# soedinglab/plass

Hardware: AMD Instinct MI355X
Metric: read-overlaps/s per assembly iteration (higher is better)
Workload: dtype u8/u64 (integer hash, byte compare; f32 ratios)

## Files before the change

### plass_amd/csrc/kmermatch.hip

```cpp
#include "common.hpp"
#include "device_utils.hpp"
#include "host_util.hpp"
#include "linepart.hpp"
#include "ref_rules.hpp"
#include "xxh64_u64.hpp"
#include <algorithm>
#include <memory>
#include <type_traits>
#include <cstdlib>
#include <climits>
#include <cstring>

namespace plasship {

#include "kmermatch_extract.hpp"
#include "kmermatch_group.hpp"
#include "kmermatch_repsort.hpp"
}
using namespace plasship;

namespace {

struct Timer {
    plasship_ctx *ctx; int slot;
    void start(int s) { slot = s; (void) hipEventRecord(ctx->ev[s], ctx->stream); }
    float stop(int s2) { (void) hipEventRecord(ctx->ev[s2], ctx->stream); (void) hipEventSynchronize(ctx->ev[s2]); float ms = 0; (void) hipEventElapsedTime(&ms, ctx->ev[slot], ctx->ev[s2]); return ms; }
};

static inline unsigned gridFor(uint64_t n, unsigned block, unsigned cap = 65535u * 8) {
    uint64_t g = (n + block - 1) / block; if (g < 1) g = 1; if (g > cap) g = cap; return (unsigned) g;
}
static int ceilLog2(uint64_t x) { int b = 0; while ((1ULL << b) < x) b++; return b; }

__global__ void lastRunInfoKernel(const unsigned long long *__restrict__ maxRT, const uint64_t *__restrict__ slotOff, const uint32_t *__restrict__ len,
                                  uint32_t n, unsigned long long *__restrict__ out) {
    const unsigned long long m = *maxRT;
    const uint32_t t = (uint32_t) (m & 0xFFFFFFFFull);
    out[0] = m;
    if (t < n) { out[1] = slotOff[t]; out[2] = slotOff[t + 1]; out[3] = len[t]; } else { out[1] = out[2] = out[3] = 0; }
}

template <bool LONG>
__global__ void countBadIdsKernel(const void *recs, uint64_t n, uint32_t nSeq, unsigned long long *out) {
    const Rec<LONG> *g = reinterpret_cast<const Rec<LONG> *>(recs);
    unsigned long long bad = 0, sen = 0;
    for (uint64_t i = (uint64_t) blockIdx.x * blockDim.x + threadIdx.x; i < n; i += (uint64_t) gridDim.x * blockDim.x) {
        const Rec<LONG> r = g[i];
        if (isSentinel(r)) sen++; else if (r.id >= nSeq) bad++;
    }
    if (bad) atomicAdd(&out[0], bad);
    if (sen) atomicAdd(&out[1], sen);
}
template <bool LONG>
static void traceBadIds(plasship_ctx *ctx, const char *what, const void *recs, uint64_t n, uint32_t nSeq) {
    if (!traceOn()) return;
    DevBuf d; unsigned long long h[2] = {0, 0};
    if (d.alloc(16) != hipSuccess) return;
    (void) hipMemsetAsync(d.p, 0, 16, ctx->stream);
    hipLaunchKernelGGL((countBadIdsKernel<LONG>), dim3(1024), dim3(256), 0, ctx->stream, recs, n, nSeq, d.as<unsigned long long>());
    (void) hipMemcpyAsync(h, d.p, 16, hipMemcpyDeviceToHost, ctx->stream);
    const hipError_t e = plasship::streamSync(ctx->stream);
    fprintf(stderr, "[plasship] %s: %llu records, %llu with an id out of range, %llu sentinels (%s)\n", what, (unsigned long long) n, h[0], h[1], hipGetErrorString(e));
}

__global__ void splitIdsKernel(const uint64_t *__restrict__ slotOff, uint32_t n, int W, uint64_t *__restrict__ out) {
    const uint64_t total = slotOff[n];
    for (int r = threadIdx.x; r <= W; r += blockDim.x) {
        uint32_t lo = 0, hi = n;
        if (r == W) lo = n;
        else {
            const uint64_t want = (uint64_t) (((unsigned __int128) total * (unsigned) r) / (unsigned) W);
            while (lo < hi) { const uint32_t mid = lo + (hi - lo) / 2; if (slotOff[mid] < want) lo = mid + 1; else hi = mid; }
        }
        out[r] = lo; out[W + 1 + r] = slotOff[lo];
    }
}

struct LineGeo {
    int b1 = 0, b2 = 0; uint32_t nb1 = 1, nb2 = 0, PL1 = 1, PL2 = 0;
    uint64_t totalLines = 0, nP1 = 0, cap1 = 0, maxP2 = 0, cap2 = 0;
    uint32_t lastValid = RPL;
};
static uint32_t pieceLinesFor(uint64_t lines, uint32_t nb, int numCU, uint32_t minFactor) {
    const uint64_t want = (lines + 4ull * (uint64_t) numCU - 1) / (4ull * (uint64_t) numCU);
    return (uint32_t) std::max<uint64_t>((uint64_t) nb * minFactor, std::min<uint64_t>((uint64_t) nb * 64, std::max<uint64_t>(want, 1)));
}
static LineGeo lineGeometry(uint64_t totalSlots, bool lng, int numCU, uint64_t slotsAll = 0, int W = 1) {
    LineGeo g;
    const int maxBits = lng ? 9 : 10;
    const int lw = ceilLog2((uint64_t) std::max(W, 1));
    int totalBits = std::min(2 * maxBits, std::max(lw, std::max(0, ceilLog2(((slotsAll ? slotsAll : totalSlots) + 1535) / 1536))));
    if (const char *pb = getenv("PLASSHIP_TUNE_PART_BITS")) { if (*pb) totalBits = std::min(2 * maxBits, std::max(lw, atoi(pb))); }
    g.b1 = totalBits <= maxBits ? totalBits : std::max((totalBits + 1) / 2, lw); g.b2 = totalBits - g.b1;
    g.nb1 = 1u << g.b1; g.nb2 = g.b2 ? 1u << g.b2 : 0u;
    g.totalLines = (totalSlots + RPL - 1) / RPL;
    g.lastValid = g.totalLines ? (uint32_t) (totalSlots - (g.totalLines - 1) * RPL) : (uint32_t) RPL;
    g.PL1 = pieceLinesFor(g.totalLines, g.nb1, numCU, 8);
    g.nP1 = (g.totalLines + g.PL1 - 1) / g.PL1;
    g.cap1 = std::max<uint64_t>(g.nP1 * ((uint64_t) g.PL1 + g.nb1), 1);
    if (g.nb2) {
        g.PL2 = 0xFFFFFFFFu; g.maxP2 = g.nb1; g.cap2 = g.cap1 + (uint64_t) g.nb1 * g.nb2;
    }
    return g;
}
static uint64_t repLevel1Cap(uint64_t nRec, uint64_t nSeg, uint32_t PL, uint32_t nb) {
    const uint64_t lines = (nRec + RPL - 1) / RPL + nSeg;
    return lines + (lines / PL + nSeg + 1) * (uint64_t) nb;
}

__global__ void arenaStartKernel(const uint32_t *__restrict__ lineBeg, uint32_t bpb, uint32_t gGrid, uint32_t nBuckets, uint64_t *__restrict__ arenaStart) {
    for (uint32_t j = blockIdx.x * blockDim.x + threadIdx.x; j < gGrid; j += gridDim.x * blockDim.x)
        arenaStart[j] = (uint64_t) lineBeg[std::min(j * bpb, nBuckets - 1)] * RPL;
}
__global__ void bigNeedKernel(const uint32_t *__restrict__ lineCnt, const uint32_t *__restrict__ unique, uint32_t nBuckets, uint64_t *__restrict__ need, uint32_t wordsPerEntry) {
    for (uint32_t b = blockIdx.x * blockDim.x + threadIdx.x; b < nBuckets; b += gridDim.x * blockDim.x) {
        const uint64_t c = (uint64_t) lineCnt[b] * RPL;
        uint64_t v = 0;
        if (unique[b] == AGG_NEEDS_SCRATCH) { uint64_t P = 1; while (P < c) P <<= 1; v = wordsPerEntry * P; }
        need[b] = v;
    }
}
__global__ void sumU32Kernel(const uint32_t *__restrict__ v, uint32_t n, unsigned long long *__restrict__ out) {
    unsigned long long s = 0;
    for (uint32_t i = blockIdx.x * blockDim.x + threadIdx.x; i < n; i += gridDim.x * blockDim.x) s += v[i];
    s = waveReduceSumU64(s);
    if (laneId() == 0 && s) atomicAdd(out, s);
}

template <class K> static int setDynLds(K k, size_t bytes) {
    PH_CHECK(hipFuncSetAttribute(reinterpret_cast<const void *>(k), hipFuncAttributeMaxDynamicSharedMemorySize, (int) bytes));
    return PLASSHIP_OK;
}
template <bool NUCL, bool LONG, int MODE, bool LIST, bool EXTRAS>
static int launchLinePart(plasship_ctx *ctx, const LinePartArgs &a, uint64_t nPiecesBound) {
    const size_t lds = linePartLdsBytes(a.nb, sizeof(Rec<LONG>), EXTRAS);
    const bool big = lds > 72 * 1024;
    const unsigned grid = (unsigned) std::max<uint64_t>(1, std::min<uint64_t>(nPiecesBound, (uint64_t) ctx->numCU * (big ? 1u : 2u)));
    if (big) {
        auto k = linePartKernel<NUCL, LONG, MODE, LIST, EXTRAS, 1024, 4, true>;
        const int rc = setDynLds(k, lds); if (rc) return rc;
        hipLaunchKernelGGL(k, dim3(grid), dim3(1024), lds, ctx->stream, a);
    } else {
        auto k = linePartKernel<NUCL, LONG, MODE, LIST, EXTRAS, 512, 4, true>;
        const int rc = setDynLds(k, lds); if (rc) return rc;
        hipLaunchKernelGGL(k, dim3(grid), dim3(512), lds, ctx->stream, a);
    }
    return PLASSHIP_OK;
}

static int buildLineLists(plasship_ctx *ctx, const uint32_t *dTags, uint64_t capLines, uint32_t nb, uint32_t *dCount, uint32_t *dStart, uint32_t *dCursor, uint32_t *dList) {
    hipStream_t st = ctx->stream;
    PH_CHECK(hipMemsetAsync(dCount, 0, (size_t) nb * 4, st));
    const unsigned g = (unsigned) std::max<uint64_t>(1, std::min<uint64_t>((capLines + 4095) / 4096, (uint64_t) ctx->numCU * 8));
    const unsigned gs = (unsigned) std::max<uint64_t>(1, std::min<uint64_t>((capLines + TS_CHUNK - 1) / TS_CHUNK, (uint64_t) ctx->numCU * 2));
    hipLaunchKernelGGL(tagHistKernel, dim3(g), dim3(256), 0, st, dTags, capLines, nb, dCount);
    hipLaunchKernelGGL(tagScanKernel, dim3(1), dim3(1024), 0, st, (const uint32_t *) dCount, nb, dStart, dCursor);
    hipLaunchKernelGGL(tagScatterKernel, dim3(gs), dim3(TS_BLOCK), 0, st, dTags, capLines, nb, dCursor, dList);
    return PLASSHIP_OK;
}

static bool shardOwnerFiltered(int W) { const int m = tuneInt("SHARD_EXTRACT", 0); return m == 2 || (m != 1 && W <= 4); }

constexpr int KM_RETRY_EARLY_OVERFLOW_CHECK = -1000;
struct LinesOut { void *triples = nullptr; uint64_t nTriples = 0, Nk = 0, Nm = 0; std::vector<int64_t> stalePos; uint32_t staleT = 0; float msSort1 = 0, msGroup = 0, msSort2 = 0, msPart = 0; int nPart = 1;
                  uint64_t exchangedRecordBytes = 0, exchangedTripleBytes = 0; };

constexpr uint64_t HALO_SLACK = 1u << 16;

static bool aggHistOn() { return getenv("PLASSHIP_DEBUG_AGGHIST") != nullptr; }
static int aggHistRecord(hipStream_t st, const uint32_t *dLineCnt, const uint32_t *dUnique, uint32_t nSort) {
    static int call = 0;
    std::vector<uint32_t> lc(nSort), uq(nSort);
    PH_COPY_SYNC(st, lc.data(), dLineCnt, (size_t) nSort * 4, hipMemcpyDeviceToHost);
    PH_COPY_SYNC(st, uq.data(), dUnique, (size_t) nSort * 4, hipMemcpyDeviceToHost);
    constexpr int NB = 10;
    auto bin = [](uint64_t v) { if (!v) return 0; int k = 1; uint64_t e = 64; while (k < NB - 1 && v > e) { e <<= 1; k++; } return k; };
    uint64_t hr[NB] = {}, hd[NB] = {}, sr = 0, sd = 0, mr = 0, md = 0, big = 0;
    for (uint32_t b = 0; b < nSort; b++) {
        const uint64_t r = (uint64_t) lc[b] * RPL; hr[bin(r)]++; sr += r; mr = std::max(mr, r);
        if (uq[b] == AGG_NEEDS_SCRATCH) { big++; continue; }
        hd[bin(uq[b])]++; sd += uq[b]; md = std::max<uint64_t>(md, uq[b]);
    }
    std::string s = "aggHist call " + std::to_string(call++) + " buckets " + std::to_string(nSort) + " | bins 0,<=64,<=128,...,<=8192,>8192 | slots";
    for (int k = 0; k < NB; k++) s += " " + std::to_string(hr[k]);
    s += " (mean " + std::to_string(nSort ? sr / nSort : 0) + ", max " + std::to_string(mr) + ") | distinct";
    for (int k = 0; k < NB; k++) s += " " + std::to_string(hd[k]);
    s += " (mean " + std::to_string(nSort ? sd / nSort : 0) + ", max " + std::to_string(md) + ", scratch " + std::to_string(big) + ")";
    fprintf(stderr, "%s\n", s.c_str());
    return PLASSHIP_OK;
}

constexpr int GW_BLOCK = 512; constexpr uint32_t GW_HT = 4096;
static bool groupHistOn() { return getenv("PLASSHIP_DEBUG_GROUPHIST") != nullptr; }
template <bool NUCL, bool LONG>
static int groupHistRecord(hipStream_t st, const char *kernel, uint32_t regCap, uint32_t maxKeys, uint32_t nBuckets, uint32_t bpb, const uint32_t *dFineBeg, const uint32_t *dFineCnt,
                           const uint32_t *dList, const void *dRecs, uint64_t capLines) {
    typedef Rec<LONG> R;
    static int call = 0;
    std::vector<uint32_t> beg(nBuckets), cnt(nBuckets);
    if (nBuckets) { PH_COPY_SYNC(st, beg.data(), dFineBeg, (size_t) nBuckets * 4, hipMemcpyDeviceToHost); PH_COPY_SYNC(st, cnt.data(), dFineCnt, (size_t) nBuckets * 4, hipMemcpyDeviceToHost); }
    uint64_t listEnd = 0;
    for (uint32_t b = 0; b < nBuckets; b++) if (cnt[b]) listEnd = std::max<uint64_t>(listEnd, (uint64_t) beg[b] + cnt[b]);
    if (listEnd > capLines) { setError("kmermatch: groupHist: a bucket's line list ends behind the list"); return PLASSHIP_ERR_DEVICE; }
    std::vector<uint32_t> list(listEnd); std::vector<R> recs((size_t) capLines * RPL);
    if (listEnd) PH_COPY_SYNC(st, list.data(), dList, (size_t) listEnd * 4, hipMemcpyDeviceToHost);
    if (listEnd) PH_COPY_SYNC(st, recs.data(), dRecs, recs.size() * sizeof(R), hipMemcpyDeviceToHost);
    enum { EMPTY = 0, REGS = 1, BIG = 2 };
    static const char *const CLS[3] = {"empty", "regs", "big"};
    auto cls = [&](uint32_t b) { const uint64_t n = (uint64_t) cnt[b] * RPL; return n == 0 ? EMPTY : (regCap == 0 || n <= regCap) ? REGS : BIG; };
    uint64_t maxPos = 0, over = 0, maxDistinct = 0, maxSub = nBuckets ? 1 : 0, multiSub = 0, pairs[3][3] = {}, bigFirst = 0, bigLater = 0, records = 0;
    std::vector<unsigned long long> keys, per;
    for (uint32_t b = 0; b < nBuckets; b++) {
        const uint64_t n = (uint64_t) cnt[b] * RPL;
        maxPos = std::max(maxPos, n);
        if (cls(b) == BIG) { over++; (b % bpb == 0 ? bigFirst : bigLater)++; }
        if (b % bpb != 0) pairs[cls(b - 1)][cls(b)]++;
        keys.clear();
        for (uint32_t l = 0; l < cnt[b]; l++) {
            const uint64_t line = list[beg[b] + l];
            if (line >= capLines) { setError("kmermatch: groupHist: a line list entry is out of range"); return PLASSHIP_ERR_DEVICE; }
            for (int i = 0; i < RPL; i++) { const R &r = recs[line * RPL + i]; if (!(r.kmer == ~0ULL && r.id == 0xFFFFFFFFu)) keys.push_back(NUCL ? (r.kmer | BIT63) : r.kmer); }
        }
        records += keys.size();
        std::sort(keys.begin(), keys.end()); keys.erase(std::unique(keys.begin(), keys.end()), keys.end());
        maxDistinct = std::max<uint64_t>(maxDistinct, keys.size());
        uint32_t nSub = 1;
        for (;; nSub *= 2) {
            per.assign(nSub, 0);
            for (const unsigned long long K : keys) per[(uint32_t) (((K * 0xD6E8FEB86659FD93ULL) >> 40) % nSub)]++;
            if (*std::max_element(per.begin(), per.end()) <= maxKeys) break;
        }
        maxSub = std::max<uint64_t>(maxSub, nSub); multiSub += nSub > 1;
    }
    std::string s = "groupHist call " + std::to_string(call++) + " kernel " + kernel + " buckets " + std::to_string(nBuckets) + " bpb " + std::to_string(bpb) + " records " + std::to_string(records) +
                    " | maxPos " + std::to_string(maxPos) + " regCap " + std::to_string(regCap) + " overRegs " + std::to_string(over) + " (first " + std::to_string(bigFirst) + ", later " + std::to_string(bigLater) + ")" +
                    " | maxDistinct " + std::to_string(maxDistinct) + " maxKeys " + std::to_string(maxKeys) + " | maxSub " + std::to_string(maxSub) + " multiSub " + std::to_string(multiSub) + " | pairs";
    for (int p = 0; p < 3; p++) for (int q = 0; q < 3; q++) s += std::string(" ") + CLS[p] + ">" + CLS[q] + " " + std::to_string(pairs[p][q]);
    fprintf(stderr, "%s\n", s.c_str());
    return PLASSHIP_OK;
}

template <bool NUCL, bool LONG, bool TRIPLES, bool ORDOUT = false>
static int repSortLines(plasship_ctx *ctx, const void *in, const std::vector<std::pair<uint64_t, uint64_t>> &segs, uint64_t nIn, uint32_t nReps, uint32_t repBase, uint32_t nTargets,
                        uint64_t slackTriples, const std::function<void()> &inputConsumed, DevBuf &dOut, uint64_t &nTriples, DevBuf *dRepStartOut) {
    constexpr bool PL = TRIPLES ? NUCL : LONG;
    typedef Rec<PL> R;
    typedef typename std::conditional<ORDOUT, TripleX, Triple>::type OutT;
    hipStream_t st = ctx->stream;
    const int numCU = ctx->numCU;
    const int maxBits = PL ? 9 : 10;
    const int idBits = std::max(1, ceilLog2((uint64_t) nTargets));
    const int repBits = std::max(1, ceilLog2((uint64_t) std::max<uint32_t>(nReps, 1)));
    const int wantBits = std::min(2 * maxBits, std::max(0, ceilLog2((nIn + 511) / 512)));
    const int allowedLocal = 62 - idBits - DiagPack<LONG>::BITS;
    const int sBits = std::max(std::min(wantBits, repBits), std::max(0, repBits - allowedLocal));
    if (sBits > 2 * maxBits) { setError("kmermatch: too many sequences for the packed rep-sort key"); return PLASSHIP_ERR_UNSUPPORTED; }
    const int s1 = sBits <= maxBits ? sBits : (sBits + 1) / 2, s2 = sBits - s1;
    const uint32_t nS1 = 1u << s1, nS2 = s2 ? 1u << s2 : 0u, nSort = 1u << sBits;
    std::vector<LinePiece> hp; uint64_t outLine = 0;
    {
        uint64_t totLines = 0; for (const auto &sg : segs) totLines += (sg.second + RPL - 1) / RPL;
        const uint32_t PLr1 = pieceLinesFor(totLines, nS1, numCU, 8);
        for (const auto &sg : segs) {
            const uint64_t cnt = sg.second, lines = (cnt + RPL - 1) / RPL;
            for (uint64_t l0 = 0; l0 < lines; l0 += PLr1) {
                LinePiece pc; pc.in0 = sg.first + l0; pc.nLines = (uint32_t) std::min<uint64_t>(PLr1, lines - l0);
                pc.lastValid = (l0 + pc.nLines == lines) ? (uint32_t) (cnt - (lines - 1) * RPL) : (uint32_t) RPL;
                pc.out0 = outLine; pc.outCap = pc.nLines + nS1; pc.tagBase = 0;
                outLine += pc.outCap; hp.push_back(pc);
            }
        }
    }
    const uint32_t PLr2 = s2 ? pieceLinesFor(std::max<uint64_t>(outLine, 1), nS2, numCU, 16) : 0;
    const uint64_t maxPR2 = s2 ? std::max<uint64_t>(outLine, 1) / PLr2 + nS1 + 1 : 0;
    const uint64_t capR1 = std::max<uint64_t>(outLine, 1), capR2 = s2 ? capR1 + maxPR2 * nS2 : 0;
    const uint32_t nPR1 = (uint32_t) hp.size();
    DevBuf dR1, dRTag1, dRList1, dRPieces, dRNP, dRCnt1, dRStart1, dRCur1, dR2, dRTag2, dRList2, dRPieces2, dRNP2, dRRegBeg, dRRegEnd, dRTot2, dSortBeg, dSortCnt;
    if (dR1.alloc(capR1 * RPL * sizeof(R)) != hipSuccess || dRTag1.alloc(capR1 * 4) != hipSuccess || dRList1.alloc(capR1 * 4) != hipSuccess || dRPieces.alloc(((size_t) nPR1 + 1) * sizeof(LinePiece)) != hipSuccess ||
        dRNP.alloc(4) != hipSuccess || dRCnt1.alloc(LP_MAXB * 4) != hipSuccess || dRStart1.alloc((LP_MAXB + 1) * 4) != hipSuccess || dRCur1.alloc(LP_MAXB * 4) != hipSuccess ||
        dSortBeg.alloc((size_t) nSort * 4) != hipSuccess || dSortCnt.alloc((size_t) nSort * 4) != hipSuccess) { setError("kmermatch: out of device memory for the rep sort"); return PLASSHIP_ERR_DEVICE; }
    void *hpPinned = nPR1 ? ctxPinnedTable(ctx, (size_t) nPR1 * sizeof(LinePiece)) : nullptr;
    if (hpPinned) memcpy(hpPinned, hp.data(), (size_t) nPR1 * sizeof(LinePiece));
    if (nPR1) PH_CHECK(hipMemcpyAsync(dRPieces.p, hpPinned ? hpPinned : (const void *) hp.data(), (size_t) nPR1 * sizeof(LinePiece), hipMemcpyHostToDevice, st));
    else PH_CHECK(hipMemsetAsync(dRTag1.p, 0xFF, capR1 * 4, st));
    PH_CHECK(hipMemcpyAsync(dRNP.p, &nPR1, 4, hipMemcpyHostToDevice, st));
    LineKey rkey; rkey.rangeBits = repBits; rkey.repBase = repBase; rkey.shift = s1 ? 64 - s1 : 63; rkey.scrambleBits = repBits;
    int rc;
    {
        LinePartArgs a; memset(&a, 0, sizeof(a));
        a.in = in; a.out = dR1.p; a.tags = dRTag1.as<uint32_t>(); a.pieces = dRPieces.as<LinePiece>(); a.nPieces = dRNP.as<uint32_t>(); a.nb = nS1; a.key = rkey;
        a.direct = 1;
        rc = launchLinePart<NUCL, PL, KEY_RANGE, false, false>(ctx, a, std::max<uint32_t>(nPR1, 1)); if (rc) return rc;
// ... 796 lines not shown
```

### plass_amd/csrc/kmermatch_group.hpp

```cpp
#pragma once

constexpr int GR_BLOCK = 256;
constexpr uint32_t GR_HT = 2048;
constexpr uint32_t GR_MAXKEYS = 1536;

struct GroupArgs {
    const void *in; void *out;
    const uint64_t *bucketStart;
    const uint32_t *list, *lineBeg, *lineCnt;
    uint32_t nBuckets, bucketsPerBlock;
    uint64_t *outCount;
    int includeOnlyExtendable, covMode; float covThr;
    const unsigned long long *minKey;
    unsigned long long *maxRepTarget;
};

template <bool LONG> __device__ __forceinline__ void embedOrd(Rec<LONG> &o, uint64_t memberKmerField) {
    const uint64_t K = memberKmerField & ~BIT63;
    o.kmer |= (K & 0x7FFFFFFFull) << 32;
    o.len = (decltype(o.len)) (K >> 31);
}
template <bool LONG> __device__ __forceinline__ unsigned long long ordWordOf(const Rec<LONG> &r) {
    const uint64_t K = ((r.kmer >> 32) & 0x7FFFFFFFull) | ((uint64_t) (LONG ? (uint32_t) r.len : (uint32_t) (uint16_t) r.len) << 31);
    return (K << 1) | (r.kmer >> 63);
// ... 9 lines not shown
    __shared__ uint32_t sCursor;
    typedef Rec<LONG> R;
    const R *in = reinterpret_cast<const R *>(a.in);
    R *out = reinterpret_cast<R *>(a.out);
    const uint32_t bBegin = blockIdx.x * a.bucketsPerBlock;
    const uint32_t bEnd = min(a.nBuckets, bBegin + a.bucketsPerBlock);
    if (bBegin >= a.nBuckets) { if (threadIdx.x == 0) a.outCount[blockIdx.x] = 0; return; }
    unsigned long long written = 0;
    unsigned long long maxRT = 0;
    const uint64_t arena = LINES ? (uint64_t) a.lineBeg[bBegin] * RPL : a.bucketStart[bBegin];
    const unsigned long long firstRunKey = (NUCL && a.minKey) ? *a.minKey : 0ull;
    for (uint32_t b = bBegin; b < bEnd; b++) {
        const uint64_t s0 = LINES ? 0ull : a.bucketStart[b], s1 = LINES ? (uint64_t) a.lineCnt[b] * RPL : a.bucketStart[b + 1];
        const uint32_t lb = LINES ? a.lineBeg[b] : 0u;
        auto recAt = [&](uint64_t i) -> R { if (LINES) return in[(uint64_t) a.list[lb + (uint32_t) (i / RPL)] * RPL + (i % RPL)]; return in[i]; };
        if (s1 <= s0) continue;
        uint32_t nSub = 1;
        const unsigned long long writtenAtBucketStart = written;
        for (;;) {
            bool redo = false;
            for (uint32_t sub = 0; sub < nSub && !redo; sub++) {
                for (uint32_t i = threadIdx.x; i < GR_HT; i += GR_BLOCK) { hKey[i] = ~0ULL; hBest[i] = ~0ULL; hCnt[i] = 0; hLen[i] = 0; }
                if (threadIdx.x == 0) { sFlag[0] = 0; sFlag[1] = 0; sCursor = 0; }
                __syncthreads();
                for (uint64_t i = s0 + threadIdx.x; i < s1; i += GR_BLOCK) {
                    const R r = recAt(i);
                    if (LINES && isSentinel(r)) continue;
                    const unsigned long long K = NUCL ? (r.kmer | BIT63) : r.kmer;
                    const uint64_t hh = K * 0xD6E8FEB86659FD93ULL;
                    if (nSub > 1 && (uint32_t) ((hh >> 40) % nSub) != sub) continue;
                    uint32_t slot = (uint32_t) (hh >> 32) & (GR_HT - 1);
                    for (uint32_t probe = 0; probe < GR_HT; probe++) {
                        const unsigned long long prev = atomicCAS(&hKey[slot], ~0ULL, K);
                        if (prev == ~0ULL) { atomicAdd(&sFlag[0], 1u); }
                        if (prev == ~0ULL || prev == K) { atomicAdd(&hCnt[slot], 1u); atomicMax(&hLen[slot], (uint32_t) r.len); break; }
                        slot = (slot + 1) & (GR_HT - 1);
                        if (probe == GR_HT - 1) atomicExch(&sFlag[1], 1u);
                    }
                }
                __syncthreads();
                if (sFlag[1] || sFlag[0] > GR_MAXKEYS) { redo = true; __syncthreads(); break; }
                for (uint64_t i = s0 + threadIdx.x; i < s1; i += GR_BLOCK) {
                    const R r = recAt(i);
                    if (LINES && isSentinel(r)) continue;
                    const unsigned long long K = NUCL ? (r.kmer | BIT63) : r.kmer;
                    const uint64_t hh = K * 0xD6E8FEB86659FD93ULL;
                    if (nSub > 1 && (uint32_t) ((hh >> 40) % nSub) != sub) continue;
                    uint32_t slot = (uint32_t) (hh >> 32) & (GR_HT - 1);
                    while (hKey[slot] != K) slot = (slot + 1) & (GR_HT - 1);
                    if ((uint32_t) r.len == hLen[slot]) {
                        const unsigned long long packed = ((unsigned long long) r.id << 22) | ((unsigned long long) (uint32_t) r.pos << 1) | (NUCL ? ((r.kmer >> 63) & 1ULL) : 0ULL);
                        atomicMin(&hBest[slot], packed);
                    }
                }
                __syncthreads();
                for (uint64_t i0 = s0; i0 < s1; i0 += GR_BLOCK) {
                    const uint64_t i = i0 + threadIdx.x;
                    bool keep = false; R o; memset(&o, 0, sizeof(R));
                    if (i < s1) {
                        const R r = recAt(i);
                        const unsigned long long K = NUCL ? (r.kmer | BIT63) : r.kmer;
                        const uint64_t hh = K * 0xD6E8FEB86659FD93ULL;
                        if (!(LINES && isSentinel(r)) && !(nSub > 1 && (uint32_t) ((hh >> 40) % nSub) != sub)) {
                            uint32_t slot = (uint32_t) (hh >> 32) & (GR_HT - 1);
                            while (hKey[slot] != K) slot = (slot + 1) & (GR_HT - 1);
                            if (hCnt[slot] >= 2) {
                                const unsigned long long best = hBest[slot];
                                const uint32_t repId = (uint32_t) (best >> 22);
                                const int repPos = (int) ((best >> 1) & 0x1FFFFFu);
                                const int queryLen = (int) hLen[slot];
                                const int mLen = (int) r.len, mPos = (int) r.pos;
                                int diagonal = repPos - mPos;
                                unsigned long long rId = repId;
                                if (NUCL) {
                                    bool repIsReverse = ((best & 1ULL) == 0);
                                    if (K == firstRunKey) repIsReverse = false;
                                    const bool targetIsReverse = ((r.kmer & BIT63) == 0);
                                    int qp, tp; bool qRev;
                                    if (repIsReverse && !targetIsReverse) { qp = repPos; tp = mPos; qRev = true; }
                                    else if (repIsReverse && targetIsReverse) { qp = (queryLen - 1) - repPos; tp = (mLen - 1) - mPos; qRev = false; }
                                    else if (!repIsReverse && targetIsReverse) { qp = (queryLen - 1) - repPos; tp = (mLen - 1) - mPos; qRev = true; }
                                    else { qp = repPos; tp = mPos; qRev = false; }
                                    if (!LONG) { qp = (int) (short) qp; tp = (int) (short) tp; }
                                    diagonal = qp - tp;
                                    rId = qRev ? (rId & ~BIT63) : (rId | BIT63);
                                }
                                const bool canBeExtended = diagonal < 0 || (diagonal > (queryLen - mLen));
                                const bool cov = canBeCovered(a.covThr, a.covMode, (float) queryLen, (float) mLen);
                                keep = (!a.includeOnlyExtendable && cov) || (canBeExtended && a.includeOnlyExtendable);
                                o.kmer = rId; o.id = r.id; o.len = r.len; o.pos = (decltype(o.pos)) diagonal;
                                if (NUCL) embedOrd(o, r.kmer);
                                if (keep) maxRT = max(maxRT, (unsigned long long) (((rId & ~BIT63) << 32) | (unsigned long long) r.id));
                            }
                        }
                    }
                    const unsigned long long mk = __ballot(keep);
                    const uint32_t wr = (uint32_t) __popcll(mk & ((1ULL << laneId()) - 1ULL));
                    uint32_t wbase = 0;
                    if (mk) {
                        if (laneId() == 0) wbase = atomicAdd(&sCursor, (uint32_t) __popcll(mk));
                        wbase = __shfl(wbase, 0, 64);
                    }
                    if (keep) out[arena + written + wbase + wr] = o;
                }
                __syncthreads();
                written += sCursor;
                __syncthreads();
                if (threadIdx.x == 0) sCursor = 0;
            }
            if (!redo) break;
            nSub *= 2;
            written = writtenAtBucketStart;
            __syncthreads();
        }
    }
    if (a.maxRepTarget) {
#pragma unroll
        for (int o = 32; o > 0; o >>= 1) maxRT = max(maxRT, (unsigned long long) __shfl_xor(maxRT, o, 64));
        if (laneId() == 0 && maxRT) atomicMax(a.maxRepTarget, maxRT);
    }
    if (threadIdx.x == 0) a.outCount[blockIdx.x] = written;
}

constexpr int GL_RMAX = 8;
constexpr uint32_t glMaxKeys(uint32_t HT) { return HT / 4 * 3; }
template <bool NUCL, int BLOCK, uint32_t HT, int WPE>
__global__ __launch_bounds__(BLOCK) __attribute__((amdgpu_waves_per_eu(WPE, WPE))) void groupLinesKernel(GroupArgs a) {
    __shared__ uint32_t sList[GL_RMAX * BLOCK / RPL];
    typedef Rec<false> R;
    constexpr uint32_t MAXKEYS = glMaxKeys(HT);
    __shared__ unsigned long long hKey[HT];
    __shared__ unsigned long long hBest[HT];
    __shared__ uint32_t hMulti[HT / 32];
    __shared__ uint32_t sFlag[2];
    __shared__ uint32_t sCursor[2];
    const R *in = reinterpret_cast<const R *>(a.in);
    R *out = reinterpret_cast<R *>(a.out);
    const uint32_t bBegin = blockIdx.x * a.bucketsPerBlock;
    const uint32_t bEnd = min(a.nBuckets, bBegin + a.bucketsPerBlock);
    if (bBegin >= a.nBuckets) { if (threadIdx.x == 0) a.outCount[blockIdx.x] = 0; return; }
    unsigned long long written = 0;
    unsigned long long maxRT = 0;
    const uint64_t arena = (uint64_t) a.lineBeg[bBegin] * RPL;
    const unsigned long long firstRunKey = (NUCL && a.minKey) ? *a.minKey : 0ull;
    const R none = [] { R r; r.kmer = ~0ULL; r.id = 0xFFFFFFFFu; r.len = 0; r.pos = 0; return r; }();
    R rg[GL_RMAX];
    uint32_t nNext = 0, lbNext = 0;
    auto fetch = [&](uint32_t b, bool fromLds) {
        nNext = (b < bEnd) ? a.lineCnt[b] * RPL : 0u; lbNext = (b < bEnd) ? a.lineBeg[b] : 0u;
        if (nNext && nNext <= (uint32_t) GL_RMAX * BLOCK) {
#pragma unroll
            for (int j = 0; j < GL_RMAX; j++) {
                const uint32_t i = (uint32_t) j * BLOCK + threadIdx.x;
                const uint32_t le = fromLds ? sList[i / RPL] : a.list[lbNext + i / RPL];
                rg[j] = (i < nNext) ? in[(uint64_t) le * RPL + (i % RPL)] : none;
            }
        }
    };
    uint32_t par = 0;
    fetch(bBegin, false);
    for (uint32_t b = bBegin; b < bEnd; b++) {
        const uint32_t n = nNext;
        const uint32_t lb = lbNext;
        if (n == 0) { fetch(b + 1, false); continue; }
        uint32_t leAhead = 0; bool aheadStored = false;
        if (b + 1 < bEnd) { const uint32_t nl = a.lineCnt[b + 1]; if (threadIdx.x < nl && nl <= (uint32_t) GL_RMAX * BLOCK / RPL) leAhead = a.list[a.lineBeg[b + 1] + threadIdx.x]; }
        auto recAt = [&](uint32_t i) -> R { return in[(uint64_t) a.list[lb + i / RPL] * RPL + (i % RPL)]; };
        const bool inRegs = n <= (uint32_t) GL_RMAX * BLOCK;
        bool fetched = false;
        auto phaseA = [&](const R &r, uint32_t nSub, uint32_t sub) {
            bool claimed = false, full = false;
            const unsigned long long K = NUCL ? (r.kmer | BIT63) : r.kmer;
            const uint64_t hh = K * 0xD6E8FEB86659FD93ULL;
            if (!isSentinel(r) && !(nSub > 1 && (uint32_t) ((hh >> 40) % nSub) != sub)) {
                uint32_t slot = (uint32_t) (hh >> 32) & (HT - 1);
                full = true;
                for (uint32_t probe = 0; probe < HT; probe++) {
                    const unsigned long long prev = atomicCAS(&hKey[slot], ~0ULL, K);
                    if (prev == ~0ULL || prev == K) {
                        claimed = (prev == ~0ULL);
                        if (!claimed) atomicOr(&hMulti[slot >> 5], 1u << (slot & 31));
                        const unsigned long long packed = ((unsigned long long) (0x7FFFu - (uint32_t) r.len) << 48) | ((unsigned long long) r.id << 16) |
                                                          ((unsigned long long) ((uint32_t) r.pos & 0x7FFFu) << 1) | (NUCL ? ((r.kmer >> 63) & 1ULL) : 0ULL);
                        atomicMin(&hBest[slot], packed);
                        full = false;
                        break;
                    }
                    slot = (slot + 1) & (HT - 1);
                }
            }
            const unsigned long long cm = __ballot(claimed);
            if (cm && laneId() == 0) atomicAdd(&sFlag[0], (uint32_t) __popcll(cm));
            if (full) atomicExch(&sFlag[1], 1u);
        };
        auto phaseC = [&](const R &r, uint32_t nSub, uint32_t sub) {
            bool keep = false; R o; o.kmer = 0; o.id = 0; o.len = 0; o.pos = 0;
            if (!isSentinel(r)) {
                const unsigned long long K = NUCL ? (r.kmer | BIT63) : r.kmer;
                const uint64_t hh = K * 0xD6E8FEB86659FD93ULL;
                if (!(nSub > 1 && (uint32_t) ((hh >> 40) % nSub) != sub)) {
                    uint32_t slot = (uint32_t) (hh >> 32) & (HT - 1);
                    while (hKey[slot] != K) slot = (slot + 1) & (HT - 1);
                    if ((hMulti[slot >> 5] >> (slot & 31)) & 1u) {
                        const unsigned long long best = hBest[slot];
                        const uint32_t repId = (uint32_t) (best >> 16);
                        const int repPos = (int) ((best >> 1) & 0x7FFFu);
                        const int queryLen = (int) (0x7FFFu - (uint32_t) (best >> 48));
                        const int mLen = (int) r.len, mPos = (int) r.pos;
                        int diagonal = repPos - mPos;
                        unsigned long long rId = repId;
                        if (NUCL) {
                            bool repIsReverse = ((best & 1ULL) == 0);
                            if (K == firstRunKey) repIsReverse = false;
                            const bool targetIsReverse = ((r.kmer & BIT63) == 0);
                            int qp, tp; bool qRev;
                            if (repIsReverse && !targetIsReverse) { qp = repPos; tp = mPos; qRev = true; }
                            else if (repIsReverse && targetIsReverse) { qp = (queryLen - 1) - repPos; tp = (mLen - 1) - mPos; qRev = false; }
                            else if (!repIsReverse && targetIsReverse) { qp = (queryLen - 1) - repPos; tp = (mLen - 1) - mPos; qRev = true; }
                            else { qp = repPos; tp = mPos; qRev = false; }
                            qp = (int) (short) qp; tp = (int) (short) tp;
                            diagonal = qp - tp;
                            rId = qRev ? (rId & ~BIT63) : (rId | BIT63);
                        }
                        const bool canBeExtended = diagonal < 0 || (diagonal > (queryLen - mLen));
                        const bool cov = canBeCovered(a.covThr, a.covMode, (float) queryLen, (float) mLen);
                        keep = (!a.includeOnlyExtendable && cov) || (canBeExtended && a.includeOnlyExtendable);
                        o.kmer = rId; o.id = r.id; o.len = r.len; o.pos = (int16_t) diagonal;
                        if (NUCL) embedOrd(o, r.kmer);
                        if (keep) maxRT = max(maxRT, (unsigned long long) (((rId & ~BIT63) << 32) | (unsigned long long) r.id));
                    }
                }
            }
            const unsigned long long mk = __ballot(keep);
            const uint32_t wr = (uint32_t) __popcll(mk & ((1ULL << laneId()) - 1ULL));
            uint32_t wbase = 0;
            if (mk) {
                if (laneId() == 0) wbase = atomicAdd(&sCursor[par], (uint32_t) __popcll(mk));
                wbase = __shfl(wbase, 0, 64);
            }
            if (keep) out[arena + written + wbase + wr] = o;
        };
        uint32_t nSub = 1;
        const unsigned long long writtenAtBucketStart = written;
        for (;;) {
            bool redo = false;
            for (uint32_t sub = 0; sub < nSub && !redo; sub++) {
                for (uint32_t i = threadIdx.x; i < HT; i += BLOCK) { hKey[i] = ~0ULL; hBest[i] = ~0ULL; if (i < HT / 32) hMulti[i] = 0; }
                if (threadIdx.x == 0) { sFlag[0] = 0; sFlag[1] = 0; sCursor[par] = 0; }
                __syncthreads();
                if (inRegs) {
#pragma unroll
                    for (int j = 0; j < GL_RMAX; j++) if ((uint32_t) j * BLOCK < n) phaseA(rg[j], nSub, sub);
                } else for (uint32_t i0 = 0; i0 < n; i0 += BLOCK) { const uint32_t i = i0 + threadIdx.x; phaseA(i < n ? recAt(i) : none, nSub, sub); }
                if (!aheadStored) { if (threadIdx.x < GL_RMAX * BLOCK / RPL) sList[threadIdx.x] = leAhead; aheadStored = true; }
                __syncthreads();
                if (sFlag[1] || sFlag[0] > MAXKEYS) { redo = true; __syncthreads(); break; }
                if (inRegs && sub + 1 == nSub) {
                    const uint32_t nN = (b + 1 < bEnd) ? a.lineCnt[b + 1] * RPL : 0u, lbN = (b + 1 < bEnd) ? a.lineBeg[b + 1] : 0u;
                    const bool nextRegs = nN && nN <= (uint32_t) GL_RMAX * BLOCK;
#pragma unroll
                    for (int j = 0; j < GL_RMAX; j++) {
                        if ((uint32_t) j * BLOCK < n) phaseC(rg[j], nSub, sub);
                        if (nextRegs) { const uint32_t i = (uint32_t) j * BLOCK + threadIdx.x; rg[j] = (i < nN) ? in[(uint64_t) sList[i / RPL] * RPL + (i % RPL)] : none; }
                    }
                    nNext = nN; lbNext = lbN; fetched = true;
                } else {
                if (inRegs) {
#pragma unroll
                    for (int j = 0; j < GL_RMAX; j++) if ((uint32_t) j * BLOCK < n) phaseC(rg[j], nSub, sub);
                } else for (uint32_t i0 = 0; i0 < n; i0 += BLOCK) { const uint32_t i = i0 + threadIdx.x; phaseC(i < n ? recAt(i) : none, nSub, sub); }
                if (sub + 1 == nSub) { fetch(b + 1, true); fetched = true; }
                }
                __syncthreads();
                written += sCursor[par];
                par ^= 1u;
            }
            if (!redo) break;
            nSub *= 2;
            written = writtenAtBucketStart;
            __syncthreads();
        }
        if (!fetched) fetch(b + 1, false);
    }
    if (a.maxRepTarget) {
#pragma unroll
        for (int o = 32; o > 0; o >>= 1) maxRT = max(maxRT, (unsigned long long) __shfl_xor(maxRT, o, 64));
        if (laneId() == 0 && maxRT) atomicMax(a.maxRepTarget, maxRT);
    }
    if (threadIdx.x == 0) a.outCount[blockIdx.x] = written;
}
```

### plass_amd/csrc/linepart.hpp

```cpp
#pragma once
#include "common.hpp"
#include "device_utils.hpp"

namespace plasship {

#define BIT63 (1ULL << 63)

template <bool LONG> struct Rec;
template <> struct __attribute__((aligned(16))) Rec<false> { uint64_t kmer; uint32_t id; uint16_t len; int16_t pos; };
template <> struct __attribute__((aligned(8))) Rec<true> { uint64_t kmer; uint32_t id; int32_t len; int32_t pos; uint32_t pad; };

template <bool LONG> __device__ __forceinline__ bool isSentinel(const Rec<LONG> &r) { return r.kmer == ~0ULL && r.id == 0xFFFFFFFFu; }

enum { KEY_HASH = 0, KEY_RANGE = 1 };
template <bool NUCL> __device__ __forceinline__ uint64_t kmerMix(uint64_t kmerField) {
    const uint64_t K = NUCL ? (kmerField & ~BIT63) : kmerField;
    uint64_t x = K * 0x9E3779B97F4A7C15ULL; x ^= x >> 29; x *= 0xBF58476D1CE4E5B9ULL; x ^= x >> 32;
    return x;
}

constexpr uint32_t VH_BINS = 2048;
template <bool NUCL> __device__ __host__ __forceinline__ uint32_t valueBin(uint64_t kmerField, int shift) {
    const uint64_t v = NUCL ? (kmerField & ~BIT63) : kmerField;
    const uint64_t b = v >> shift;
    return b < VH_BINS ? (uint32_t) b : VH_BINS - 1;
}

#ifndef PLASSHIP_RPL
#define PLASSHIP_RPL 8
#endif
constexpr int RPL = PLASSHIP_RPL;
constexpr uint32_t TAG_NONE = 0xFFFFFFFFu;
constexpr uint32_t LP_MAXB = 1024;

struct LineKey {
    int shift, rangeBits;
    uint64_t repBase;
    int scrambleBits;
};
__device__ __host__ __forceinline__ uint64_t scrambleRep(uint64_t rep, int bits) {
    uint32_t x = (uint32_t) rep;
    x = ((x >> 1) & 0x55555555u) | ((x & 0x55555555u) << 1); x = ((x >> 2) & 0x33333333u) | ((x & 0x33333333u) << 2);
    x = ((x >> 4) & 0x0F0F0F0Fu) | ((x & 0x0F0F0F0Fu) << 4); x = ((x >> 8) & 0x00FF00FFu) | ((x & 0x00FF00FFu) << 8);
    x = (x >> 16) | (x << 16);
    return (uint64_t) (x >> (32 - bits));
}
template <bool NUCL, int MODE> __device__ __forceinline__ uint32_t lineBucket(const LineKey &k, uint64_t kmerField, uint32_t nb) {
    if (MODE == KEY_HASH) return (uint32_t) (kmerMix<NUCL>(kmerField) >> k.shift) & (nb - 1);
    uint64_t r = (kmerField & ~BIT63) - k.repBase;
    if (k.scrambleBits) r = scrambleRep(r, k.scrambleBits);
    return (uint32_t) ((r << (64 - k.rangeBits)) >> k.shift) & (nb - 1);
}

struct LinePiece {
    uint64_t in0;
    uint64_t out0;
    uint32_t nLines;
    uint32_t lastValid;
    uint32_t outCap;
    uint32_t tagBase;
};

struct LinePartArgs {
    const void *in; const uint32_t *list;
    void *out; uint32_t *tags;
    const LinePiece *pieces; const uint32_t *nPieces;
    uint64_t totalLines; uint32_t lastValidAll, pieceLines;
    uint32_t *pieceOut;
    LineKey key; uint32_t nb;
    int direct;
    unsigned long long *minKey;
    uint32_t *valueHist; int valueShift;
    uint32_t keepLo, keepHi;
};

static inline size_t linePartLdsBytes(uint32_t nb, size_t recBytes, bool extras) {
    return (size_t) nb * RPL * recBytes + (size_t) nb * 8 + (extras ? VH_BINS * 4 : 0) + (size_t) nb * 2 + (size_t) nb * 4 + 16;
}

template <bool NUCL, bool LONG, int MODE, bool LIST, bool EXTRAS, int LP_BLOCK, int LP_ITEMS, bool PREFETCH>
__global__ __launch_bounds__(LP_BLOCK) void linePartKernel(LinePartArgs a) {
    constexpr int LP_TILE = LP_BLOCK * LP_ITEMS;
    typedef Rec<LONG> R;
    extern __shared__ __attribute__((aligned(16))) unsigned char lpDyn[];
    const uint32_t nb = a.nb;
    R *buf = reinterpret_cast<R *>(lpDyn);
    uint32_t *cnt = reinterpret_cast<uint32_t *>(lpDyn + (size_t) nb * RPL * sizeof(R));
    uint32_t *flushed = cnt + nb;
    uint32_t *vh = flushed + nb;
    uint32_t *lbase = vh + (EXTRAS ? VH_BINS : 0);
    unsigned short *queue = reinterpret_cast<unsigned short *>(lbase + nb);
    __shared__ uint32_t sQ[2];
    __shared__ uint32_t sScan[LP_BLOCK / 64 + 1];
    const uint32_t tid = threadIdx.x;
    const R *in = reinterpret_cast<const R *>(a.in);
    R *out = reinterpret_cast<R *>(a.out);
    if (tid < 2) sQ[tid] = 0;
    if (EXTRAS && a.valueHist) for (uint32_t i = tid; i < VH_BINS; i += LP_BLOCK) vh[i] = 0;
    unsigned long long mn = ~0ULL;
    uint32_t round = 0;
    const uint32_t nPieces = a.pieces ? *a.nPieces : (uint32_t) ((a.totalLines + a.pieceLines - 1) / a.pieceLines);
    R sen; __builtin_memset(&sen, 0xFF, sizeof(R));
    for (uint32_t piece = blockIdx.x; piece < nPieces; piece += gridDim.x) {
        LinePiece pc;
        if (a.pieces) pc = a.pieces[piece];
        else {
            pc.in0 = (uint64_t) piece * a.pieceLines;
            pc.nLines = (uint32_t) (a.totalLines - pc.in0 < (uint64_t) a.pieceLines ? a.totalLines - pc.in0 : (uint64_t) a.pieceLines);
            pc.lastValid = (pc.in0 + pc.nLines == a.totalLines) ? a.lastValidAll : (uint32_t) RPL;
            pc.out0 = (uint64_t) piece * ((uint64_t) a.pieceLines + nb); pc.outCap = a.pieceLines + nb; pc.tagBase = 0;
        }
        for (uint32_t i = tid; i < nb; i += LP_BLOCK) { cnt[i] = 0; flushed[i] = 0; }
        __syncthreads();
        uint64_t outLine = pc.out0;
        const uint64_t nRec = (uint64_t) (pc.nLines - 1) * RPL + pc.lastValid;
        R nxt[LP_ITEMS];
        uint32_t lnNext[LP_ITEMS];
        auto loadLines = [&](uint64_t t0) {
#pragma unroll
            for (int u = 0; u < LP_ITEMS; u++) {
                const uint64_t i = t0 + (uint64_t) u * LP_BLOCK + tid;
                lnNext[u] = (LIST && i < nRec) ? a.list[pc.in0 + i / RPL] : 0u;
            }
        };
        auto loadTile = [&](uint64_t t0) {
#pragma unroll
            for (int u = 0; u < LP_ITEMS; u++) {
                const uint64_t i = t0 + (uint64_t) u * LP_BLOCK + tid;
                if (i < nRec) {
                    const uint64_t line = LIST ? (uint64_t) lnNext[u] : pc.in0 + i / RPL;
                    nxt[u] = in[line * RPL + (i % RPL)];
                } else nxt[u] = sen;
            }
        };
        if (LIST) loadLines(0);
        if (PREFETCH) { loadTile(0); if (LIST) loadLines(LP_TILE); }
        for (uint64_t t0 = 0; t0 < nRec; t0 += LP_TILE) {
            R rec[LP_ITEMS]; uint32_t bk[LP_ITEMS], sq[LP_ITEMS]; uint32_t pending = 0;
            if (!PREFETCH) { loadTile(t0); if (LIST) loadLines(t0 + LP_TILE); }
#pragma unroll
            for (int u = 0; u < LP_ITEMS; u++) rec[u] = nxt[u];
            if (PREFETCH && t0 + LP_TILE < nRec) { loadTile(t0 + LP_TILE); if (LIST) loadLines(t0 + 2 * (uint64_t) LP_TILE); }
#pragma unroll
            for (int u = 0; u < LP_ITEMS; u++) {
                bk[u] = 0; sq[u] = 0;
                {
                    if (!isSentinel(rec[u])) {
                        const uint32_t b = lineBucket<NUCL, MODE>(a.key, rec[u].kmer, nb);
                        if (EXTRAS && a.keepHi && (b < a.keepLo || b >= a.keepHi)) continue;
                        bk[u] = b; sq[u] = atomicAdd(&cnt[b], 1u); pending |= 1u << u;
                        if (EXTRAS) {
                            if (a.valueHist) atomicAdd(&vh[valueBin<NUCL>(rec[u].kmer, a.valueShift)], 1u);
                            if (NUCL && a.minKey) mn = min(mn, (unsigned long long) (rec[u].kmer | BIT63));
                        }
                    }
                }
            }
            if (MODE == KEY_RANGE && a.direct) {
                __syncthreads();
                uint32_t mine = 0;
                for (uint32_t b = tid; b < nb; b += LP_BLOCK) mine += cnt[b] / RPL - flushed[b] / RPL;
                const uint32_t incl = waveInclusiveScan(mine);
                if (laneId() == 63) sScan[tid >> 6] = incl;
                __syncthreads();
                uint32_t woff = 0, total = 0;
#pragma unroll
                for (int w = 0; w < LP_BLOCK / 64; w++) { const uint32_t v = sScan[w]; if (w < (int) (tid >> 6)) woff += v; total += v; }
                uint32_t run = woff + incl - mine;
                for (uint32_t b = tid; b < nb; b += LP_BLOCK) {
                    const uint32_t oldC = flushed[b], done = cnt[b] / RPL - oldC / RPL;
                    lbase[b] = run;
                    if (done && (oldC % RPL)) {
                        const uint64_t ol = outLine + run;
                        for (uint32_t r = 0; r < oldC % RPL; r++) out[ol * RPL + r] = buf[(size_t) b * RPL + r];
                        a.tags[ol] = pc.tagBase + b;
                    }
                    run += done;
                }
                __syncthreads();
#pragma unroll
                for (int u = 0; u < LP_ITEMS; u++) {
                    if ((pending >> u) & 1u) {
                        const uint32_t b = bk[u], L = sq[u] / RPL, oldL = flushed[b] / RPL, newL = cnt[b] / RPL;
                        if (L < newL) {
                            const uint64_t ol = outLine + lbase[b] + (L - oldL);
                            out[ol * RPL + (sq[u] % RPL)] = rec[u];
                            if (sq[u] % RPL == 0) a.tags[ol] = pc.tagBase + b;
                        } else buf[(size_t) b * RPL + (sq[u] % RPL)] = rec[u];
                    }
                }
                __syncthreads();
                for (uint32_t b = tid; b < nb; b += LP_BLOCK) flushed[b] = cnt[b];
                outLine += total;
                __syncthreads();
                continue;
            }
            for (;;) {
                const uint32_t par = round & 1u;
#pragma unroll
                for (int u = 0; u < LP_ITEMS; u++) {
                    if ((pending >> u) & 1u) {
                        const uint32_t b = bk[u];
                        if (sq[u] / RPL == flushed[b]) {
                            buf[(size_t) b * RPL + (sq[u] % RPL)] = rec[u];
                            pending &= ~(1u << u);
                            if (sq[u] % RPL == RPL - 1) { const uint32_t q = atomicAdd(&sQ[par], 1u); queue[q] = (unsigned short) b; }
                        }
                    }
                }
                __syncthreads();
                const uint32_t nQ = sQ[par];
                for (uint32_t j = tid; j < nQ * RPL; j += LP_BLOCK) { const uint32_t b = queue[j / RPL]; out[(outLine + j / RPL) * RPL + (j % RPL)] = buf[(size_t) b * RPL + (j % RPL)]; }
                for (uint32_t j = tid; j < nQ; j += LP_BLOCK) { const uint32_t b = queue[j]; a.tags[outLine + j] = pc.tagBase + b; flushed[b] += 1u; }
                const int more = __syncthreads_or(pending != 0u);
                outLine += nQ;
                if (tid == 0) sQ[par] = 0;
                round++;
                if (!more) break;
            }
        }
        {
            const uint32_t par = round & 1u;
            __syncthreads();
            auto openRecords = [&](uint32_t b) { return (MODE == KEY_RANGE && a.direct) ? cnt[b] % RPL : cnt[b] - flushed[b] * RPL; };
            for (uint32_t b = tid; b < nb; b += LP_BLOCK) if (openRecords(b)) { const uint32_t q = atomicAdd(&sQ[par], 1u); queue[q] = (unsigned short) b; }
            __syncthreads();
            const uint32_t nQ = sQ[par];
            for (uint32_t j = tid; j < nQ * RPL; j += LP_BLOCK) {
                const uint32_t b = queue[j / RPL]; const uint32_t r = openRecords(b);
                out[(outLine + j / RPL) * RPL + (j % RPL)] = ((j % RPL) < r) ? buf[(size_t) b * RPL + (j % RPL)] : sen;
            }
            for (uint32_t j = tid; j < nQ; j += LP_BLOCK) a.tags[outLine + j] = pc.tagBase + queue[j];
            __syncthreads();
            outLine += nQ;
            if (tid == 0) sQ[par] = 0;
            round++;
        }
        for (uint64_t j = outLine + tid; j < pc.out0 + pc.outCap; j += LP_BLOCK) a.tags[j] = TAG_NONE;
        if (tid == 0 && a.pieceOut) a.pieceOut[piece] = (uint32_t) (outLine - pc.out0);
    }
    if (EXTRAS) {
        __syncthreads();
        if (a.valueHist) for (uint32_t i = tid; i < VH_BINS; i += LP_BLOCK) { const uint32_t c = vh[i]; if (c) atomicAdd(&a.valueHist[i], c); }
        if (NUCL && a.minKey) {
#pragma unroll
            for (int o = 32; o > 0; o >>= 1) mn = min(mn, (unsigned long long) __shfl_xor(mn, o, 64));
            if (laneId() == 0 && mn != ~0ULL) atomicMin(a.minKey, mn);
        }
    }
}

__global__ __launch_bounds__(256) void tagHistKernel(const uint32_t *__restrict__ tags, uint64_t nLines, uint32_t nb, uint32_t *__restrict__ count) {
    __shared__ uint32_t sh[LP_MAXB];
    for (uint32_t i = threadIdx.x; i < nb; i += 256) sh[i] = 0;
    __syncthreads();
    for (uint64_t i = (uint64_t) blockIdx.x * 256 + threadIdx.x; i < nLines; i += (uint64_t) gridDim.x * 256) { const uint32_t t = tags[i]; if (t != TAG_NONE) atomicAdd(&sh[t], 1u); }
    __syncthreads();
    for (uint32_t i = threadIdx.x; i < nb; i += 256) { const uint32_t c = sh[i]; if (c) atomicAdd(&count[i], c); }
}
__global__ __launch_bounds__(1024) void tagScanKernel(const uint32_t *__restrict__ count, uint32_t nb, uint32_t *__restrict__ start, uint32_t *__restrict__ cursor) {
    __shared__ uint32_t sWave[16];
    const uint32_t v = threadIdx.x < nb ? count[threadIdx.x] : 0u;
    const uint32_t incl = waveInclusiveScan(v);
    if (laneId() == 63) sWave[threadIdx.x >> 6] = incl;
    __syncthreads();
    uint32_t woff = 0;
    for (uint32_t w = 0; w < (threadIdx.x >> 6); w++) woff += sWave[w];
    const uint32_t ex = woff + incl - v;
    if (threadIdx.x < nb) { start[threadIdx.x] = ex; cursor[threadIdx.x] = ex; }
    if (threadIdx.x == nb - 1) start[nb] = ex + v;
}
constexpr int TS_BLOCK = 1024, TS_PER = 32, TS_CHUNK = TS_BLOCK * TS_PER;
__global__ __launch_bounds__(TS_BLOCK) void tagScatterKernel(const uint32_t *__restrict__ tags, uint64_t nLines, uint32_t nb, uint32_t *__restrict__ cursor, uint32_t *__restrict__ list) {
    __shared__ uint32_t sh[LP_MAXB];
    for (uint64_t c0 = (uint64_t) blockIdx.x * TS_CHUNK; c0 < nLines; c0 += (uint64_t) gridDim.x * TS_CHUNK) {
        for (uint32_t i = threadIdx.x; i < nb; i += TS_BLOCK) sh[i] = 0;
        __syncthreads();
        uint32_t t[TS_PER];
#pragma unroll
        for (int u = 0; u < TS_PER; u++) {
            const uint64_t i = c0 + (uint64_t) u * TS_BLOCK + threadIdx.x;
            t[u] = (i < nLines) ? tags[i] : TAG_NONE;
        }
#pragma unroll
        for (int u = 0; u < TS_PER; u++) if (t[u] != TAG_NONE) atomicAdd(&sh[t[u]], 1u);
        __syncthreads();
        for (uint32_t i = threadIdx.x; i < nb; i += TS_BLOCK) { const uint32_t c = sh[i]; sh[i] = c ? atomicAdd(&cursor[i], c) : 0u; }
        __syncthreads();
#pragma unroll
        for (int u = 0; u < TS_PER; u++) {
            const uint64_t i = c0 + (uint64_t) u * TS_BLOCK + threadIdx.x;
            if (t[u] != TAG_NONE) list[atomicAdd(&sh[t[u]], 1u)] = (uint32_t) i;
        }
        __syncthreads();
    }
}
__global__ void listRangesKernel(const uint32_t *__restrict__ start, uint32_t nb, uint32_t *__restrict__ beg, uint32_t *__restrict__ cnt) {
    for (uint32_t i = blockIdx.x * blockDim.x + threadIdx.x; i < nb; i += gridDim.x * blockDim.x) { beg[i] = start[i]; cnt[i] = start[i + 1] - start[i]; }
}

constexpr int TS_STAGE = 8;
__global__ __launch_bounds__(512) void tagSortRegionKernel(const uint32_t *__restrict__ tags, const uint64_t *__restrict__ regionBeg, const uint64_t *__restrict__ regionEnd,
                                                           uint32_t nRegions, uint32_t nb2, uint32_t *__restrict__ list, uint32_t *__restrict__ fineBeg, uint32_t *__restrict__ fineCnt) {
    __shared__ uint32_t sh[LP_MAXB];
    __shared__ uint32_t sWave[8];
    __shared__ uint32_t sCnt[LP_MAXB];
    __shared__ uint32_t sStage[TS_STAGE * LP_MAXB];
    for (uint32_t i = threadIdx.x; i < LP_MAXB; i += 512) sCnt[i] = 0;
    for (uint32_t g = blockIdx.x; g < nRegions; g += gridDim.x) {
        const uint64_t r0 = regionBeg[g], r1 = regionEnd[g];
        const uint32_t base = g * nb2;
        for (uint32_t i = threadIdx.x; i < nb2; i += 512) sh[i] = 0;
        __syncthreads();
        for (uint64_t i = r0 + threadIdx.x; i < r1; i += 2048) {
            uint32_t t[4];
#pragma unroll
            for (int u = 0; u < 4; u++) t[u] = (i + 512u * u < r1) ? tags[i + 512u * u] : TAG_NONE;
#pragma unroll
            for (int u = 0; u < 4; u++) if (t[u] != TAG_NONE) atomicAdd(&sh[t[u] - base], 1u);
        }
        __syncthreads();
        const uint32_t i0 = 2 * threadIdx.x, i1 = i0 + 1;
        const uint32_t c0 = i0 < nb2 ? sh[i0] : 0u, c1 = i1 < nb2 ? sh[i1] : 0u;
        const uint32_t incl = waveInclusiveScan(c0 + c1);
        if (laneId() == 63) sWave[threadIdx.x >> 6] = incl;
        __syncthreads();
        uint32_t woff = 0;
        for (uint32_t w = 0; w < (threadIdx.x >> 6); w++) woff += sWave[w];
        const uint32_t ex = (uint32_t) r0 + woff + incl - (c0 + c1);
        if (i0 < nb2) { fineBeg[base + i0] = ex; fineCnt[base + i0] = c0; sh[i0] = ex; }
        if (i1 < nb2) { fineBeg[base + i1] = ex + c0; fineCnt[base + i1] = c1; sh[i1] = ex + c0; }
        __syncthreads();
        for (uint64_t i0 = r0; i0 < r1; i0 += 2048) {
            const uint64_t i = i0 + threadIdx.x;
            uint32_t t[4];
#pragma unroll
            for (int u = 0; u < 4; u++) t[u] = (i + 512u * u < r1) ? tags[i + 512u * u] : TAG_NONE;
#pragma unroll
            for (int u = 0; u < 4; u++) if (t[u] != TAG_NONE) {
                const uint32_t b = t[u] - base, k = atomicAdd(&sCnt[b], 1u);
                if (k < (uint32_t) TS_STAGE) sStage[k * LP_MAXB + b] = (uint32_t) (i + 512u * u); else list[sh[b] + k] = (uint32_t) (i + 512u * u);
            }
            __syncthreads();
            for (uint32_t b = threadIdx.x; b < nb2; b += 512) {
                const uint32_t c = sCnt[b];
                if (c >= (uint32_t) TS_STAGE) {
                    uint32_t row[TS_STAGE];
#pragma unroll
                    for (int j = 0; j < TS_STAGE; j++) row[j] = sStage[j * LP_MAXB + b];
                    __builtin_memcpy(list + sh[b], row, sizeof(row));
                    sh[b] += c; sCnt[b] = 0;
                }
            }
            __syncthreads();
        }
        for (uint32_t b = threadIdx.x; b < nb2; b += 512) {
            const uint32_t c = sCnt[b], p = sh[b];
            for (uint32_t j = 0; j < c; j++) list[p + j] = sStage[j * LP_MAXB + b];
            sCnt[b] = 0;
        }
        __syncthreads();
    }
}

__device__ __forceinline__ void blockScan1024(uint32_t a, uint64_t b, uint32_t &exA, uint64_t &exB, uint32_t &totA, uint64_t &totB, uint32_t *sA, unsigned long long *sB) {
    const uint32_t inA = waveInclusiveScan(a); const unsigned long long inB = waveInclusiveScanU64(b);
    const uint32_t w = threadIdx.x >> 6;
    if (laneId() == 63) { sA[w] = inA; sB[w] = inB; }
    __syncthreads();
    uint32_t oa = 0, ta = 0; unsigned long long ob = 0, tb = 0;
#pragma unroll
    for (uint32_t k = 0; k < 16; k++) { if (k < w) { oa += sA[k]; ob += sB[k]; } ta += sA[k]; tb += sB[k]; }
    exA = oa + inA - a; exB = ob + inB - b; totA = ta; totB = tb;
    __syncthreads();
}
__global__ __launch_bounds__(1024) void planListKernel(const uint32_t *__restrict__ start, uint32_t nb1, uint32_t pieceLines, uint32_t nb2,
// ... 65 lines not shown
```

Before: 727.8 million.

## Defer line-partition flush rounds and use nontemporal loads/stores for hash mode

For the large-LDS hash-key path, the line-partition kernel now exits its flush loop once no pending record is more than one line ahead, deferring the remaining records to the buffer. It also uses nontemporal vector loads and stores for streaming records, and halves items per thread for non-list hash launches. This aims to cut barrier-heavy flush rounds and avoid cache pollution. The deferred path adds a reset of the queue counter and depends on the subsequent tail flush handling leftovers correctly. The group kernel also masks list reads beyond the bucket size.

```diff
diff --git a/plass_amd/csrc/kmermatch.hip b/plass_amd/csrc/kmermatch.hip
--- a/plass_amd/csrc/kmermatch.hip
+++ b/plass_amd/csrc/kmermatch.hip
@@ -137,7 +137,8 @@
     const bool big = lds > 72 * 1024;
     const unsigned grid = (unsigned) std::max<uint64_t>(1, std::min<uint64_t>(nPiecesBound, (uint64_t) ctx->numCU * (big ? 1u : 2u)));
     if (big) {
-        auto k = linePartKernel<NUCL, LONG, MODE, LIST, EXTRAS, 1024, 4, true>;
+        constexpr bool HASH = MODE == KEY_HASH;
+        auto k = linePartKernel<NUCL, LONG, MODE, LIST, EXTRAS, 1024, (HASH && !LIST) ? 2 : 4, true, HASH, HASH>;
         const int rc = setDynLds(k, lds); if (rc) return rc;
         hipLaunchKernelGGL(k, dim3(grid), dim3(1024), lds, ctx->stream, a);
     } else {
diff --git a/plass_amd/csrc/kmermatch_group.hpp b/plass_amd/csrc/kmermatch_group.hpp
--- a/plass_amd/csrc/kmermatch_group.hpp
+++ b/plass_amd/csrc/kmermatch_group.hpp
@@ -185,7 +185,7 @@
 #pragma unroll
             for (int j = 0; j < GL_RMAX; j++) {
                 const uint32_t i = (uint32_t) j * BLOCK + threadIdx.x;
-                const uint32_t le = fromLds ? sList[i / RPL] : a.list[lbNext + i / RPL];
+                const uint32_t le = (i < nNext) ? (fromLds ? sList[i / RPL] : a.list[lbNext + i / RPL]) : 0u;
                 rg[j] = (i < nNext) ? in[(uint64_t) le * RPL + (i % RPL)] : none;
             }
         }
diff --git a/plass_amd/csrc/linepart.hpp b/plass_amd/csrc/linepart.hpp
--- a/plass_amd/csrc/linepart.hpp
+++ b/plass_amd/csrc/linepart.hpp
@@ -78,7 +78,31 @@
     return (size_t) nb * RPL * recBytes + (size_t) nb * 8 + (extras ? VH_BINS * 4 : 0) + (size_t) nb * 2 + (size_t) nb * 4 + 16;
 }
 
-template <bool NUCL, bool LONG, int MODE, bool LIST, bool EXTRAS, int LP_BLOCK, int LP_ITEMS, bool PREFETCH>
+template <class R> __device__ __forceinline__ R streamLoad(const R *p) {
+    if constexpr (sizeof(R) == 16 && alignof(R) == 16) {
+        typedef uint32_t V __attribute__((ext_vector_type(4)));
+        const V v = __builtin_nontemporal_load(reinterpret_cast<const V *>(p));
+        R r; __builtin_memcpy(&r, &v, sizeof(R)); return r;
+    } else {
+        uint64_t w[sizeof(R) / 8];
+#pragma unroll
+        for (size_t k = 0; k < sizeof(R) / 8; k++) w[k] = __builtin_nontemporal_load(reinterpret_cast<const uint64_t *>(p) + k);
+        R r; __builtin_memcpy(&r, w, sizeof(R)); return r;
+    }
+}
+template <class R> __device__ __forceinline__ void streamStore(R *p, const R &r) {
+    if constexpr (sizeof(R) == 16 && alignof(R) == 16) {
+        typedef uint32_t V __attribute__((ext_vector_type(4)));
+        V v; __builtin_memcpy(&v, &r, sizeof(R));
+        __builtin_nontemporal_store(v, reinterpret_cast<V *>(p));
+    } else {
+        uint64_t w[sizeof(R) / 8]; __builtin_memcpy(w, &r, sizeof(R));
+#pragma unroll
+        for (size_t k = 0; k < sizeof(R) / 8; k++) __builtin_nontemporal_store(w[k], reinterpret_cast<uint64_t *>(p) + k);
+    }
+}
+
+template <bool NUCL, bool LONG, int MODE, bool LIST, bool EXTRAS, int LP_BLOCK, int LP_ITEMS, bool PREFETCH, bool DEFER = false, bool NT = false>
 __global__ __launch_bounds__(LP_BLOCK) void linePartKernel(LinePartArgs a) {
     constexpr int LP_TILE = LP_BLOCK * LP_ITEMS;
     typedef Rec<LONG> R;
@@ -129,7 +153,7 @@
                 const uint64_t i = t0 + (uint64_t) u * LP_BLOCK + tid;
                 if (i < nRec) {
                     const uint64_t line = LIST ? (uint64_t) lnNext[u] : pc.in0 + i / RPL;
-                    nxt[u] = in[line * RPL + (i % RPL)];
+                    nxt[u] = NT ? streamLoad(in + line * RPL + (i % RPL)) : in[line * RPL + (i % RPL)];
                 } else nxt[u] = sen;
             }
         };
@@ -197,31 +221,51 @@
             }
             for (;;) {
                 const uint32_t par = round & 1u;
+                bool far = false;
 #pragma unroll
                 for (int u = 0; u < LP_ITEMS; u++) {
                     if ((pending >> u) & 1u) {
-                        const uint32_t b = bk[u];
-                        if (sq[u] / RPL == flushed[b]) {
+                        const uint32_t b = bk[u], f = flushed[b];
+                        if (sq[u] / RPL == f) {
                             buf[(size_t) b * RPL + (sq[u] % RPL)] = rec[u];
                             pending &= ~(1u << u);
                             if (sq[u] % RPL == RPL - 1) { const uint32_t q = atomicAdd(&sQ[par], 1u); queue[q] = (unsigned short) b; }
-                        }
+                        } else if (sq[u] / RPL > f + 1) far = true;
                     }
                 }
                 __syncthreads();
                 const uint32_t nQ = sQ[par];
-                for (uint32_t j = tid; j < nQ * RPL; j += LP_BLOCK) { const uint32_t b = queue[j / RPL]; out[(outLine + j / RPL) * RPL + (j % RPL)] = buf[(size_t) b * RPL + (j % RPL)]; }
+                for (uint32_t j = tid; j < nQ * RPL; j += LP_BLOCK) {
+                    const uint32_t b = queue[j / RPL];
+                    if (NT) streamStore(out + (outLine + j / RPL) * RPL + (j % RPL), buf[(size_t) b * RPL + (j % RPL)]);
+                    else out[(outLine + j / RPL) * RPL + (j % RPL)] = buf[(size_t) b * RPL + (j % RPL)];
+                }
                 for (uint32_t j = tid; j < nQ; j += LP_BLOCK) { const uint32_t b = queue[j]; a.tags[outLine + j] = pc.tagBase + b; flushed[b] += 1u; }
-                const int more = __syncthreads_or(pending != 0u);
+                const int more = __syncthreads_or(DEFER ? far : pending != 0u);
                 outLine += nQ;
                 if (tid == 0) sQ[par] = 0;
                 round++;
                 if (!more) break;
             }
+            if (DEFER) {
+                const uint32_t par = round & 1u;
+#pragma unroll
+                for (int u = 0; u < LP_ITEMS; u++) {
+                    if ((pending >> u) & 1u) {
+                        const uint32_t b = bk[u];
+                        buf[(size_t) b * RPL + (sq[u] % RPL)] = rec[u];
+                        if (sq[u] % RPL == RPL - 1) { const uint32_t q = atomicAdd(&sQ[par], 1u); queue[q] = (unsigned short) b; }
+                    }
+                }
+            }
         }
         {
             const uint32_t par = round & 1u;
             __syncthreads();
+            if (DEFER) {
+                if (tid == 0) sQ[par] = 0;
+                __syncthreads();
+            }
             auto openRecords = [&](uint32_t b) { return (MODE == KEY_RANGE && a.direct) ? cnt[b] % RPL : cnt[b] - flushed[b] * RPL; };
             for (uint32_t b = tid; b < nb; b += LP_BLOCK) if (openRecords(b)) { const uint32_t q = atomicAdd(&sQ[par], 1u); queue[q] = (unsigned short) b; }
             __syncthreads();
```

After: 747.9 million, median of 6. +2.8%, better.
